# kiliant/zklaim

Measured on AMD Instinct MI355X. Metric: Groth16 proofs/sec (zklaim gadget, alt_bn128) + G1 MSM GB/s vs HBM roofline, higher is better.
Workload: dtype u32 limbs, Montgomery (254-bit Fq/Fr: 9 x 29-bit in the accumulation, reduction and NTT kernels, 8 x 32-bit elsewhere)

## Files before the change

zklaim_amd/csrc/msm.hip:

```cpp
#include "common.hpp"
#include "fq29.hip.hpp"
#include "../../include/zkg.h"
#include <algorithm>
#include <chrono>
#include <cstdio>
#include <cstdlib>
#include <cstring>
#include <mutex>

#define ZK_VGPR_CAP(n) __attribute__((amdgpu_num_vgpr((n) / 2)))
static constexpr int ACC29_VGPRS = 192;

namespace zk {

static constexpr int SCALAR_BITS = 255;
template <class F> struct RedGeom { static constexpr int LANES_LOG = sizeof(F) == sizeof(Fq) ? 7 : 6, LANES = 1 << LANES_LOG, THREADS = 4 * LANES; };
static constexpr int RED_L_LOG_TINY = 0, RED_L_LOG_SMALL = 2, RED_L_LOG_LARGE = 4;
static constexpr size_t RED_SMALL_BUCKETS = (size_t)1 << 16, RED_LARGE_BUCKETS = (size_t)1 << 18;
static constexpr int MAX_C = 16;
static constexpr uint32_t HEAVY_S = 512;
static constexpr uint32_t HEAVY_T_MAX = 1024;
static constexpr int HEAVY_PART_BLOCKS = 512, HEAVY_MERGE_BLOCKS = 128;
static constexpr int SORT_THREADS = 1024;
static constexpr int SCAN_ITEMS = 4;
// ... 253 lines not shown
    extern __shared__ uint32_t lds_u32[];
    const uint32_t s = blockIdx.x, w = blockIdx.y, t = threadIdx.x;
    const uint32_t *rel = hist + ((size_t)w * S + s) * B, *off = offsets + (size_t)w * B;
    for (uint32_t b = t; b < B; b += SORT_THREADS) lds_u32[b] = off[b] + rel[b];
    __syncthreads();
    size_t lo = (size_t)s * slice_len, hi = lo + slice_len < n ? lo + slice_len : n;
    const uint32_t *d = digits + (size_t)w * n;
    for (size_t i = lo + t; i < hi; i += SORT_THREADS) {
        uint32_t code = d[i];
        if (code) { uint32_t pos = atomicAdd(&lds_u32[(code >> 1) - 1], 1u); sorted[pos] = ((uint32_t)i << 1) | (code & 1u); }
    }
}


static constexpr uint32_t RX_MAX_CBITS = 10, RX_MAX_CB = 1u << RX_MAX_CBITS, RX_SLICE = 16384, RX_PER_THREAD = 16, RX_FINE_MAX = 8192, RX_BIN_AVG = 4096;
__global__ __launch_bounds__(1024) void k_rx_count(const uint32_t *digits, size_t n, uint32_t fbits, uint32_t cbits, uint32_t *cnt) {
    sort_wave_priority();
    __shared__ uint32_t c[RX_MAX_CB];
    const uint32_t sl = blockIdx.x, w = blockIdx.y, t = threadIdx.x, CB = 1u << cbits;
    if (t < CB) c[t] = 0;
    __syncthreads();
    size_t lo = (size_t)sl * RX_SLICE, hi = lo + RX_SLICE < n ? lo + RX_SLICE : n;
    const uint32_t *d = digits + (size_t)w * n;
    if ((n & 3) == 0) {
        for (size_t i = lo + 4 * t; i < hi; i += 4096) {
            const uint4 q = *reinterpret_cast<const uint4 *>(d + i);
            if (q.x) atomicAdd(&c[((q.x >> 1) - 1) >> fbits], 1u);
            if (q.y) atomicAdd(&c[((q.y >> 1) - 1) >> fbits], 1u);
            if (q.z) atomicAdd(&c[((q.z >> 1) - 1) >> fbits], 1u);
            if (q.w) atomicAdd(&c[((q.w >> 1) - 1) >> fbits], 1u);
        }
    } else
    for (size_t i = lo + t; i < hi; i += 1024) { uint32_t code = d[i]; if (code) atomicAdd(&c[((code >> 1) - 1) >> fbits], 1u); }
    __syncthreads();
    if (t < CB && c[t]) atomicAdd(&cnt[w * CB + t], c[t]);
}
__global__ __launch_bounds__(1024) void k_rx_scan(const uint32_t *cnt, uint32_t nbins, uint32_t *base, uint32_t *cursor, uint32_t *grand_total) {
    sort_wave_priority();
    __shared__ uint32_t part[1024];
    const uint32_t t = threadIdx.x, per = (nbins + 1023) / 1024, lo = t * per, hi = lo + per < nbins ? lo + per : nbins;
    uint32_t sum = 0;
    for (uint32_t i = lo; i < hi; ++i) sum += cnt[i];
    part[t] = sum;
    __syncthreads();
    for (uint32_t d = 1; d < 1024; d <<= 1) {
        uint32_t x = (t >= d) ? part[t - d] : 0;
        __syncthreads();
        part[t] += x;
        __syncthreads();
    }
    uint32_t run = part[t] - sum;
    for (uint32_t i = lo; i < hi; ++i) { base[i] = run; cursor[i] = 0; run += cnt[i]; }
    if (t == 1023) { base[nbins] = part[1023]; *grand_total = part[1023]; }
}
template <int T>
__global__ __launch_bounds__(T) void k_rx_scatter(const uint32_t *digits, size_t n, uint32_t fbits, uint32_t cbits, const uint32_t *base, uint32_t *cursor,
                                                   uint32_t *tmp) {
    sort_wave_priority();
    extern __shared__ uint32_t lds_u32[];
    constexpr uint32_t SLICE = RX_PER_THREAD * T;
    const uint32_t CB = 1u << cbits;
    uint32_t *stage = lds_u32, *c = lds_u32 + SLICE, *off = c + RX_MAX_CB, *gb = off + RX_MAX_CB + 1, *cur = gb + RX_MAX_CB;
    const uint32_t sl = blockIdx.x, w = blockIdx.y, t = threadIdx.x;
    for (uint32_t b = t; b < CB; b += T) c[b] = 0;
    __syncthreads();
    size_t lo = (size_t)sl * SLICE, hi = lo + SLICE < n ? lo + SLICE : n;
    const uint32_t *d = digits + (size_t)w * n;
// ... 121 lines not shown
        bufB[of[f] + atomicAdd(&cur[f], 1u)] = e & low;
    }
    __syncthreads();
    for (uint32_t p = t; p < cnt; p += T) sorted[start + p] = bufB[p];
}

ZK_D uint32_t heavy_threshold_dev(const uint32_t *offsets, size_t total_buckets, uint32_t divisor) {
    uint32_t entries = offsets[total_buckets];
    uint32_t avg6 = (uint32_t)(6 * (uint64_t)entries / total_buckets), slack = 8 + avg6 > 32 ? 32 : 8 + avg6;
    uint32_t t = (uint32_t)(4 * (uint64_t)entries / total_buckets) + slack;
    t = t > HEAVY_T_MAX ? HEAVY_T_MAX : t;
    t /= divisor;
    return t < 4 ? 4 : t;
}

__global__ __launch_bounds__(1024) void k_class_hist(const uint32_t *counts, const uint32_t *offsets, size_t total, uint32_t *class_hist) {
    sort_wave_priority();
    __shared__ uint32_t h[HEAVY_T_MAX + 2];
    const uint32_t heavy_t = heavy_threshold_dev(offsets, total, 1);
    const uint32_t t = threadIdx.x, nc = heavy_t + 2;
    for (uint32_t i = t; i < nc; i += 1024) h[i] = 0;
    __syncthreads();
    size_t gb = (size_t)blockIdx.x * 1024 + t;
    if (gb < total) { uint32_t c = counts[gb]; atomicAdd(&h[c > heavy_t ? heavy_t + 1 : c], 1u); }
    __syncthreads();
    for (uint32_t i = t; i < nc; i += 1024) if (h[i]) atomicAdd(&class_hist[i], h[i]);
}
__global__ __launch_bounds__(1024) void k_class_scan(uint32_t *class_hist, const uint32_t *offsets, size_t total) {
    sort_wave_priority();
    __shared__ uint32_t part[1024];
    const uint32_t heavy_t = heavy_threshold_dev(offsets, total, 1), nc = heavy_t + 2, t = threadIdx.x;
    uint32_t v0 = 2 * t < nc ? class_hist[nc - 1 - 2 * t] : 0, v1 = 2 * t + 1 < nc ? class_hist[nc - 2 - 2 * t] : 0;
    part[t] = v0 + v1;
    __syncthreads();
    for (uint32_t d = 1; d < 1024; d <<= 1) {
        uint32_t x = (t >= d) ? part[t - d] : 0;
        __syncthreads();
        part[t] += x;
        __syncthreads();
    }
    const uint32_t before = part[t] - v0 - v1;
    if (2 * t < nc) class_hist[nc - 1 - 2 * t] = before;
    if (2 * t + 1 < nc) class_hist[nc - 2 - 2 * t] = before + v0;
}
__global__ __launch_bounds__(1024) void k_order_place(const uint32_t *counts, const uint32_t *offsets, size_t total, uint32_t *class_cursor, uint32_t *order) {
    sort_wave_priority();
    __shared__ uint32_t h[HEAVY_T_MAX + 2];
    const uint32_t heavy_t = heavy_threshold_dev(offsets, total, 1);
    const uint32_t t = threadIdx.x, nc = heavy_t + 2;
    for (uint32_t i = t; i < nc; i += 1024) h[i] = 0;
    __syncthreads();
    size_t gb = (size_t)blockIdx.x * 1024 + t;
    uint32_t cls = 0, rank = 0;
    if (gb < total) { uint32_t c = counts[gb]; cls = c > heavy_t ? heavy_t + 1 : c; rank = atomicAdd(&h[cls], 1u); }
    __syncthreads();
    for (uint32_t i = t; i < nc; i += 1024) if (h[i]) h[i] = atomicAdd(&class_cursor[i], h[i]);
    __syncthreads();
    if (gb < total) order[h[cls] + rank] = (uint32_t)gb;
}

template <class F, bool PLAIN>
__global__ __launch_bounds__(256) void k_bucket_accum(const ViewSet<F> views, const uint32_t *sorted, const uint32_t *offsets, const uint32_t *order,
                                                       size_t lanes , XYZZ<F> *buckets, HeavyItem *items,
                                                       HeavyBucket *heavy, uint32_t *counters , SetLayout L) {
    size_t tid = (size_t)blockIdx.x * blockDim.x + threadIdx.x;
    if (tid >= lanes) return;
    const size_t total_buckets = L.buckets;
    const uint32_t set = blockIdx.y;
    const BaseView<F> bases = views.v[set];
    buckets += set * L.buckets; items += set * L.items; heavy += set * L.heavy; counters += 2 * set;
    const uint32_t heavy_t = heavy_threshold_dev(offsets, total_buckets, sizeof(F) > sizeof(Fq) ? 3 : 1);
    const uint32_t gb = order[tid];
    uint32_t k = offsets[gb], end = offsets[gb + 1];
// ... 28 lines not shown
}
ZK_D Affine29 load29(const Rec64 *bases, uint32_t e) { return load_rec64(bases + (e >> 1)); }
ZK_D Rec64 load29_raw(const Rec64 *bases, uint32_t e) { return load_rec64_raw(bases + (e >> 1)); }
template <int WAVES, bool OUT29>
__global__ __launch_bounds__(256, WAVES) ZK_VGPR_CAP(ACC29_VGPRS) void k_bucket_accum29(const Rec64 *bases, size_t level_stride, uint32_t B, const uint32_t *sorted, const uint32_t *offsets, const uint32_t *order,
                                                         size_t lanes, void *buckets_, HeavyItem *items, HeavyBucket *heavy, uint32_t *counters, SetLayout L, int flags ) {
    crit_wave_priority(flags & 2);
    const int resume = flags & 1;
    size_t tid = (size_t)blockIdx.x * blockDim.x + threadIdx.x;
    if (tid >= lanes) return;
    const uint32_t heavy_t = heavy_threshold_dev(offsets, L.buckets, 1);
    const uint32_t gb = order[tid];
    if (level_stride) bases += (size_t)(gb / B) * level_stride;
    uint32_t k = offsets[gb], end = offsets[gb + 1];
    if (end - k > heavy_t) {
        uint32_t nparts = (end - k + HEAVY_S - 1) / HEAVY_S;
        uint32_t first = atomicAdd(&counters[0], nparts);
        const bool single = nparts == 1 && !resume;
        for (uint32_t p = 0; p < nparts; ++p) { uint32_t a = k + p * HEAVY_S; items[first + p] = {a, a + HEAVY_S < end ? a + HEAVY_S : end, gb, single}; }
        if (!single) heavy[atomicAdd(&counters[1], 1u)] = {gb, first, nparts};
        return;
    }
    XYZZ29 acc; bool inf = true;
    acc.x = acc.y = acc.zz = acc.zzz = Fq29::zero();
    if constexpr (OUT29) {
        if (resume) {
            if (k >= end) return;
            const Bucket29 old = load_bucket29_raw(reinterpret_cast<const Bucket29 *>(buckets_) + gb);
            uint32_t any = 0;
#pragma unroll
// ... 542 lines not shown
};
struct MsmJob {
    hipStream_t stream = nullptr; bool own_stream = false;
    DevBuf digits, hist, counts, offsets, scan_sums, class_hist, order, sorted, rx_tmp, rx_meta;
    MsmGroup group[2];
    MsmGeom g{}; size_t n = 0;
    int window_hint = 0;
    uint32_t merge_hint = 1, merge = 1;
    hipStream_t aux = nullptr; hipEvent_t ev_fork = nullptr, ev_join = nullptr; bool converted_aside = false;
    bool one_pass_sort = false;
    bool resume = false, defer_reduce = false; bool last_out29 = false;
    hipEvent_t ev_tail = nullptr; bool tail_recorded = false;
    bool critical = false;
    MsmJob *bucket_owner = nullptr;
    hipStream_t sort_stream = nullptr; hipEvent_t ev_sorted = nullptr, ev_acc_done = nullptr;
    uint32_t w0 = 0, ws = 1;
    bool empty = false;
    uint32_t multi = 1; size_t multi_stride = 0;
    DevBuf hs_scalars; hipStream_t copy = nullptr; hipEvent_t ev_piece[8] = {nullptr};
    std::mutex mu;
};

template <class F>
static int launch_accumulate(MsmJob *job, MsmGroup &gr, const MsmBases *sets, const uint32_t *d_gather, bool time_it) {
    const MsmGeom g = job->g; const size_t n = job->n, total_buckets = (size_t)g.W * g.B; const unsigned ns = (unsigned)gr.nsets;
    const uint32_t P = job->multi, BP = g.B * P, Wp = g.W / P;
    hipStream_t s = job->stream;
    size_t n_entries_max = n * g.W;
    const size_t max_heavy = std::min(total_buckets, n_entries_max / (sizeof(F) != sizeof(Fq) ? 4 : 8)) + 1,
                 max_items = max_heavy + n_entries_max / HEAVY_S + 1;
    typedef RedGeom<F> RG;
    gr.table = sets[0].level_stride != 0;
    gr.red_windows = gr.table ? P : g.W;
    const size_t red_buckets = (size_t)gr.red_windows * g.B;
    static const char *force_l = getenv("ZKG_RED_L_LOG");
    const int red_l_log = force_l ? atoi(force_l) : red_buckets >= RED_LARGE_BUCKETS ? RED_L_LOG_LARGE : red_buckets > RED_SMALL_BUCKETS ? RED_L_LOG_SMALL : RED_L_LOG_TINY;
    gr.chunk_log = RG::LANES_LOG + red_l_log;
    gr.cpw = (g.B + (1u << gr.chunk_log) - 1) >> gr.chunk_log; gr.nred = (size_t)gr.red_windows * gr.cpw;
    DevBuf &bucket_buf = job->bucket_owner ? job->bucket_owner->group[sizeof(F) != sizeof(Fq) ? 1 : 0].buckets : gr.buckets;
    gr.red_slots = 2;
    SetLayout L; L.buckets = total_buckets; L.items = max_items; L.heavy = max_heavy; L.partials = max_items; L.folded = BP; L.red_out = gr.nred * 3;
    if (gr.heavy_items.reserve(ns * max_items * sizeof(HeavyItem)) || gr.heavy_buckets.reserve(ns * max_heavy * sizeof(HeavyBucket)) ||
        gr.heavy_counters.reserve(8 * MSM_MAX_SETS) || gr.heavy_partials.reserve(ns * max_items * sizeof(XYZZ<F>)) ||
        bucket_buf.reserve(ns * total_buckets * std::max(sizeof(XYZZ<F>), sizeof(Bucket29))) || gr.red_out.reserve(ns * L.red_out * sizeof(XYZZ<F>)) || ((gr.red_stride = L.red_out), false) ||
        (gr.table && gr.folded.reserve(ns * (size_t)BP * std::max(sizeof(XYZZ<F>), sizeof(Bucket29)))) || gr.host_reserve(ns * L.red_out * sizeof(XYZZ<F>))) return ZKG_ERROR;
// ... 19 lines not shown
                    hipLaunchKernelGGL(k_bases_to29, dim3((unsigned)((n + 255) / 256)), dim3(256), 0, s, reinterpret_cast<const Affine<Fq> *>(sets[0].p), n, gr.bases29.as<Rec64>());
                }
                rec29 = gr.bases29.as<Rec64>();
            }
        } else if (ns == 1 && !accum32 && !d_gather && sets[0].p29 && !sets[0].remap && sets[0].index_sub == 0) {
            use29 = true; rec29 = reinterpret_cast<const Rec64 *>(sets[0].p29); stride29 = sets[0].level_stride;
        }
    }
    static const bool red32_env = getenv("ZKG_REDUCE_32") != nullptr;
    static const bool fold32_env = getenv("ZKG_FOLD_32") != nullptr;
    const bool out29 = use29 && !red32_env && (stride29 == 0 ? !gr.table : (gr.table && ns == 1 && Wp <= 8 && !fold32_env));
    const int resume = job->resume ? 1 : 0;
    MsmJob *owner = job->bucket_owner ? job->bucket_owner : job;
    if (resume && !(out29 && owner->last_out29)) { set_error("msm: a piece can only continue 29-bit buckets"); return ZKG_ERROR; }
    owner->last_out29 = out29;
    if (time_it) g_dominant_timer.begin(s);
    bool done_ba = false;
    if constexpr (sizeof(F) == sizeof(Fq)) {
        const char *e_ba = getenv("ZKG_ACCUM_BA"), *e_k = getenv("ZKG_BA_K");
        const int ba_levels = e_ba ? std::max(0, std::min((int)ba::MAX_LEVELS, atoi(e_ba))) : 0;
        const int ba_k = e_k ? std::max(2, std::min(32, atoi(e_k) & ~1)) : 16;
        if (use29 && out29 && stride29 == 0 && !resume && ba_levels > 0 && n_entries_max >= 4096) {
            const int R = ba_levels, K = ba_k;
            const size_t per_wg = (size_t)ba::THREADS * K, words_start = n_entries_max / 32 + 2;
            size_t stride[ba::MAX_LEVELS + 1] = {0}, plane_words = 0, grid1 = 0;
            for (int l = 1; l <= R; ++l) {
                const size_t nodes = (n_entries_max >> l) + 1, grid = (nodes + per_wg - 1) / per_wg;
                stride[l] = grid * per_wg;
                plane_words += 18 * stride[l];
                if (l == 1) grid1 = grid;
// ... 17 lines not shown
                }
            }
            hipLaunchKernelGGL(k_bucket_accum_ba, dim3((unsigned)((lanes + 255) / 256)), dim3(256), 0, s, rec29, job->sorted.as<uint32_t>(), pl, R, job->offsets.as<uint32_t>(),
                               job->order.as<uint32_t>(), lanes, reinterpret_cast<Bucket29 *>(buckets), gr.heavy_items.as<HeavyItem>(), gr.heavy_buckets.as<HeavyBucket>(),
                               gr.heavy_counters.as<uint32_t>(), L);
            done_ba = true;
        }
    }
    if (done_ba) {}
    else if constexpr (sizeof(F) == sizeof(Fq)) {
        static const int waves_env = getenv("ZKG_ACC29_WAVES") ? atoi(getenv("ZKG_ACC29_WAVES")) : 0;
        const int waves29 = waves_env ? waves_env : (job->sort_stream || gr.table || job->bucket_owner) ? 2 : 3;
        auto launch29 = [&](auto kern) {
            hipLaunchKernelGGL(kern, dim3((unsigned)((lanes + 255) / 256)), dim3(256), 0, s, rec29, stride29, BP, job->sorted.as<uint32_t>(),
                               job->offsets.as<uint32_t>(), job->order.as<uint32_t>(), lanes, (void *)buckets, gr.heavy_items.as<HeavyItem>(),
                               gr.heavy_buckets.as<HeavyBucket>(), gr.heavy_counters.as<uint32_t>(), L, resume | (job->critical ? 2 : 0));
        };
        if (use29 && waves29 == 3) { if (out29) launch29(k_bucket_accum29<3, true>); else launch29(k_bucket_accum29<3, false>); }
        else if (use29) { if (out29) launch29(k_bucket_accum29<2, true>); else launch29(k_bucket_accum29<2, false>); }
    }
    if (use29 || done_ba) {}
    else if (plain)
        hipLaunchKernelGGL((k_bucket_accum<F, true>), dim3((unsigned)((lanes + 255) / 256), ns), dim3(256), 0, s,
                           views, job->sorted.as<uint32_t>(), job->offsets.as<uint32_t>(), job->order.as<uint32_t>(), lanes, buckets,
                           gr.heavy_items.as<HeavyItem>(), gr.heavy_buckets.as<HeavyBucket>(), gr.heavy_counters.as<uint32_t>(), L);
    else
        hipLaunchKernelGGL((k_bucket_accum<F, false>), dim3((unsigned)((lanes + 255) / 256), ns), dim3(256), 0, s,
                           views, job->sorted.as<uint32_t>(), job->offsets.as<uint32_t>(), job->order.as<uint32_t>(), lanes, buckets,
                           gr.heavy_items.as<HeavyItem>(), gr.heavy_buckets.as<HeavyBucket>(), gr.heavy_counters.as<uint32_t>(), L);
    if (time_it) g_dominant_timer.end(s);
    if (!job->defer_reduce && host_pool_prewake_enabled()) {
        if (!job->ev_tail && hipEventCreateWithFlags(&job->ev_tail, hipEventDisableTiming) != hipSuccess) job->ev_tail = nullptr;
        job->tail_recorded = job->ev_tail && hipEventRecord(job->ev_tail, s) == hipSuccess;
    }
    hipLaunchKernelGGL(k_heavy_parts<F>, dim3(HEAVY_PART_BLOCKS, ns), dim3(256), 256 * sizeof(LdsPoint<F>), s,
                       views, job->sorted.as<uint32_t>(), gr.heavy_items.as<HeavyItem>(), gr.heavy_counters.as<uint32_t>(), gr.heavy_partials.as<XYZZ<F>>(), buckets, L, (int)out29);
    hipLaunchKernelGGL(k_heavy_merge<F>, dim3(HEAVY_MERGE_BLOCKS, ns), dim3(256), 256 * sizeof(LdsPoint<F>), s,
                       gr.heavy_buckets.as<HeavyBucket>(), gr.heavy_counters.as<uint32_t>(), gr.heavy_partials.as<XYZZ<F>>(), buckets, L, (int)out29, resume);
    if (job->defer_reduce) {
        if (hipGetLastError() != hipSuccess) { set_error("msm kernel launch failed"); return ZKG_ERROR; }
        return ZKG_OK;
    }
    const XYZZ<F> *red_in = buckets; size_t in_stride = L.buckets;
    bool folded29 = false;
    if constexpr (sizeof(F) == sizeof(Fq)) {
        if (gr.table && out29) {
            hipLaunchKernelGGL(k_bucket_fold29, dim3((2 * BP + 255) / 256), dim3(256), 0, s, reinterpret_cast<const Bucket29 *>(buckets), job->counts.as<uint32_t>(), Wp, BP,
                               gr.folded.as<Bucket29>(), job->critical ? 1 : 0);
            red_in = gr.folded.as<XYZZ<F>>(); in_stride = L.folded; folded29 = true;
        }
    }
    if (gr.table && !folded29) {
        uint32_t slots = 1; while (slots < Wp && slots < 32) slots <<= 1;
// ... 106 lines not shown
    return acc;
}

static int sort_digits(MsmJob *job, const uint32_t *d_scalars, bool mont, const uint32_t *d_gather) {
    const MsmGeom g0 = job->g; const size_t n0 = job->n;
    if (job->merge > 1) { job->g.W /= job->merge; job->g.Wt = job->g.W; job->n *= job->merge; }
    if (job->multi > 1) { job->g.W *= job->multi; job->g.Wt = job->g.W; }
    const MsmGeom g = job->g; const size_t n = job->n;
    hipStream_t s = job->sort_stream ? job->sort_stream : job->stream;
    const size_t total = (size_t)g.W * g.B;
    uint32_t slice_len = (uint32_t)std::min<size_t>(65536, std::max<size_t>(4096, ((n + 15) / 16 + 1023) / 1024 * 1024));
    uint32_t S = (uint32_t)std::max<size_t>(1, (n + slice_len - 1) / slice_len);
    size_t nblk = (total + 1024 * SCAN_ITEMS - 1) / (1024 * SCAN_ITEMS);
    if (nblk > 1024) { set_error("msm: too many buckets for the block scan"); return ZKG_ERROR; }
    if (job->digits.reserve(std::max<size_t>(1, n * g.W) * 4) || job->hist.reserve((size_t)g.W * S * g.B * 4) || job->counts.reserve(total * 4) ||
        job->offsets.reserve((total + 1) * 4) || job->scan_sums.reserve(1024 * 4) || job->class_hist.reserve((HEAVY_T_MAX + 2) * 4) ||
        job->order.reserve(total * 4) || job->sorted.reserve(std::max<size_t>(1, n * g.W) * 4)) return ZKG_ERROR;
    uint32_t *digits = job->digits.as<uint32_t>(), *hist = job->hist.as<uint32_t>(), *counts = job->counts.as<uint32_t>(),
             *offsets = job->offsets.as<uint32_t>(), *sums = job->scan_sums.as<uint32_t>(), *chist = job->class_hist.as<uint32_t>();
    static const bool radix_off = getenv("ZKG_SORT_ONE_PASS") != nullptr;
    uint32_t cbits = 6;
    static const uint32_t bin_avg = getenv("ZKG_RX_AVG") ? (uint32_t)atoi(getenv("ZKG_RX_AVG")) : RX_BIN_AVG;
    while (cbits < RX_MAX_CBITS && cbits + 1 < g.c - 1 && (n >> cbits) > bin_avg) ++cbits;
    const bool two_pass = !radix_off && !job->one_pass_sort && g.c >= 12 && n >= 49152 && (n >> cbits) <= RX_FINE_MAX && n <= ((size_t)1 << (31 - (g.c - 1 - cbits)));
    {
        ZeroList zl{};
        int k = 0;
        zl.p[k] = chist; zl.words[k++] = HEAVY_T_MAX + 2;
        for (MsmGroup &gr : job->group) if (gr.nsets) {
            if (gr.heavy_counters.reserve(8 * MSM_MAX_SETS)) return ZKG_ERROR;
            zl.p[k] = gr.heavy_counters.as<uint32_t>(); zl.words[k++] = 2 * MSM_MAX_SETS;
        }
        if (two_pass) {
            const uint32_t nbins = g.W << cbits;
            if (job->rx_meta.reserve((3 * (size_t)nbins + 8) * 4)) return ZKG_ERROR;
            zl.p[k] = job->rx_meta.as<uint32_t>(); zl.words[k++] = 3 * nbins + 8;
        }
        static const bool generic_digits = getenv("ZKG_DIGITS_GENERIC") != nullptr;
        const dim3 dg((unsigned)((n0 + 255) / 256));
        const bool four = !d_gather && (n0 & 3) == 0 && g0.w0 == 0 && g0.ws == 1 && g0.W == g0.Wt;
        const dim3 dg4((unsigned)((n0 / 4 + 255) / 256));
        if (job->multi > 1) {
            const dim3 dgm(dg.x, job->multi);
            if (g0.c == 16) hipLaunchKernelGGL(k_digits_multi<16>, dgm, dim3(256), 0, s, d_scalars, job->multi_stride, n0, (int)mont, job->merge, digits, zl);
            else if (g0.c == 12) hipLaunchKernelGGL(k_digits_multi<12>, dgm, dim3(256), 0, s, d_scalars, job->multi_stride, n0, (int)mont, job->merge, digits, zl);
            else hipLaunchKernelGGL(k_digits_multi_any, dgm, dim3(256), 0, s, d_scalars, job->multi_stride, n0, (int)mont, g0, job->merge, digits, zl);
        }
        else if (!generic_digits && four && g0.c == 16) hipLaunchKernelGGL(k_digits_c4<16>, dg4, dim3(256), 0, s, d_scalars, n0, (int)mont, g0, digits, zl);
        else if (!generic_digits && four && g0.c == 12) hipLaunchKernelGGL(k_digits_c4<12>, dg4, dim3(256), 0, s, d_scalars, n0, (int)mont, g0, digits, zl);
        else if (!generic_digits && g0.c == 16) hipLaunchKernelGGL(k_digits_c<16>, dg, dim3(256), 0, s, d_scalars, d_gather, n0, (int)mont, g0, digits, zl);
        else if (!generic_digits && g0.c == 12) hipLaunchKernelGGL(k_digits_c<12>, dg, dim3(256), 0, s, d_scalars, d_gather, n0, (int)mont, g0, digits, zl);
        else hipLaunchKernelGGL(k_digits, dg, dim3(256), 0, s, d_scalars, d_gather, n0, (int)mont, g0, digits, zl);
    }
    if (two_pass) {
        const uint32_t fbits = g.c - 1 - cbits, CB = 1u << cbits, nbins = g.W * CB, S1 = (uint32_t)((n + RX_SLICE - 1) / RX_SLICE);
        if (job->rx_tmp.reserve(n * g.W * 4) || job->rx_meta.reserve((3 * (size_t)nbins + 8) * 4)) return ZKG_ERROR;
        uint32_t *cnt = job->rx_meta.as<uint32_t>(), *base = cnt + nbins, *cursor = base + nbins + 1, *tmp = job->rx_tmp.as<uint32_t>();
        hipLaunchKernelGGL(k_rx_count, dim3(S1, g.W), dim3(1024), 0, s, digits, n, fbits, cbits, cnt);
        hipLaunchKernelGGL(k_rx_scan, dim3(1), dim3(1024), 0, s, cnt, nbins, base, cursor, offsets + total);
        static const int wg_env = getenv("ZKG_SORT_WG") ? atoi(getenv("ZKG_SORT_WG")) : 0;
        const bool half = (wg_env ? wg_env == 512 : job->sort_stream != nullptr) && fbits <= 9;
        if (half) {
            const uint32_t S2 = (uint32_t)((n + 512 * RX_PER_THREAD - 1) / (512 * RX_PER_THREAD));
            hipLaunchKernelGGL(k_rx_scatter<512>, dim3(S2, g.W), dim3(512), (512 * RX_PER_THREAD + 4 * RX_MAX_CB + 8) * 4, s, digits, n, fbits, cbits, base, cursor, tmp);
            hipLaunchKernelGGL(k_rx_fine<512>, dim3(CB, g.W), dim3(512), (RX_FINE_MAX + 3 * (1u << fbits)) * 4, s, tmp, fbits, cbits, g.B, base, counts, offsets,
                               job->sorted.as<uint32_t>());
        } else {
            hipLaunchKernelGGL(k_rx_scatter<1024>, dim3(S1, g.W), dim3(1024), (RX_SLICE + 4 * RX_MAX_CB + 8) * 4, s, digits, n, fbits, cbits, base, cursor, tmp);
            hipLaunchKernelGGL(k_rx_fine<1024>, dim3(CB, g.W), dim3(1024), (RX_FINE_MAX + 3 * (1u << fbits)) * 4, s, tmp, fbits, cbits, g.B, base, counts, offsets,
                               job->sorted.as<uint32_t>());
        }
    } else {
    hipLaunchKernelGGL(k_hist, dim3(S, g.W), dim3(SORT_THREADS), g.B * 4, s, digits, n, g.B, S, slice_len, hist);
    hipLaunchKernelGGL(k_colscan, dim3((unsigned)((total + 255) / 256)), dim3(256), 0, s, hist, g.B, S, total, counts);
    hipLaunchKernelGGL(k_scan_blocks, dim3((unsigned)nblk), dim3(1024), 0, s, counts, offsets, sums, total);
    hipLaunchKernelGGL(k_scan_sums, dim3(1), dim3(1024), 0, s, sums, (uint32_t)nblk, offsets + total);
    hipLaunchKernelGGL(k_scan_apply, dim3((unsigned)nblk), dim3(1024), 0, s, offsets, sums, total);
    hipLaunchKernelGGL(k_place, dim3(S, g.W), dim3(SORT_THREADS), g.B * 4, s, digits, n, g.B, S, slice_len, hist, offsets, job->sorted.as<uint32_t>());
    }
    hipLaunchKernelGGL(k_class_hist, dim3((unsigned)((total + 1023) / 1024)), dim3(1024), 0, s, counts, offsets, total, chist);
    hipLaunchKernelGGL(k_class_scan, dim3(1), dim3(1024), 0, s, chist, offsets, total);
    hipLaunchKernelGGL(k_order_place, dim3((unsigned)((total + 1023) / 1024)), dim3(1024), 0, s, counts, offsets, total, chist, job->order.as<uint32_t>());
    if (hipGetLastError() != hipSuccess) { set_error("msm sort launch failed"); return ZKG_ERROR; }
    return ZKG_OK;
}

MsmJob *msm_job_create(hipStream_t s, bool own_stream, bool high_priority) {
    MsmJob *j = new MsmJob();
    j->stream = s;
    if (own_stream) {
        int prio_lo = 0, prio_hi = 0;
        (void)hipDeviceGetStreamPriorityRange(&prio_lo, &prio_hi);
        if (!hip_ok(hipStreamCreateWithPriority(&j->stream, hipStreamNonBlocking, high_priority ? prio_hi : prio_lo), "hipStreamCreate", __FILE__, __LINE__)) { delete j; return nullptr; }
        j->own_stream = true;
    }
    return j;
}
// ... 47 lines not shown
    {
        static const bool accum32 = getenv("ZKG_ACCUM_32") != nullptr, inline29 = getenv("ZKG_TO29_INLINE") != nullptr;
        MsmGroup &g1 = job->group[0];
        if (!accum32 && !inline29 && !any_table && !d_gather && g1.nsets == 1 && by_field[0][0].index_sub == 0 && !by_field[0][0].remap && !by_field[0][0].p29) {
            if (!job->aux && (hipStreamCreateWithFlags(&job->aux, hipStreamNonBlocking) != hipSuccess || hipEventCreateWithFlags(&job->ev_fork, hipEventDisableTiming) != hipSuccess ||
                              hipEventCreateWithFlags(&job->ev_join, hipEventDisableTiming) != hipSuccess)) { set_error("msm: side stream"); return ZKG_ERROR; }
            if (g1.bases29.reserve(n * sizeof(Rec64))) return ZKG_ERROR;
            ZK_HIP(hipEventRecord(job->ev_fork, job->stream));
            ZK_HIP(hipStreamWaitEvent(job->aux, job->ev_fork, 0));
            hipLaunchKernelGGL(k_bases_to29, dim3((unsigned)((n + 255) / 256)), dim3(256), 0, job->aux, reinterpret_cast<const Affine<Fq> *>(by_field[0][0].p), n, g1.bases29.as<Rec64>());
            ZK_HIP(hipEventRecord(job->ev_join, job->aux));
            job->converted_aside = true;
        }
    }
    auto fail = [&] { if (job->converted_aside) { (void)hipStreamSynchronize(job->aux); job->converted_aside = false; } return ZKG_ERROR; };
    if (sort_digits(job, d_scalars, scalars_mont, d_gather)) return fail();
    if (job->sort_stream && job->sort_stream != job->stream) {
        if (hipEventRecord(job->ev_sorted, job->sort_stream) != hipSuccess || hipStreamWaitEvent(job->stream, job->ev_sorted, 0) != hipSuccess) return fail();
    }
    if (job->merge > 1) {
        for (int k = 0; k < 2; ++k) for (int i = 0; i < job->group[k].nsets; ++i) by_field[k][i].level_stride *= job->merge;
    }
    lap("sort enqueued");
    const bool timed_field_g2 = job->group[0].nsets == 0;
    if (job->group[1].nsets && launch_accumulate<Fq2>(job, job->group[1], by_field[1], d_gather, job == &g_default_job && timed_field_g2)) return fail();
    if (job->group[0].nsets && launch_accumulate<Fq>(job, job->group[0], by_field[0], d_gather, job == &g_default_job || job == &g_piece_job)) return fail();
    lap("accum enqueued");
    return ZKG_OK;
}
bool msm_multi_supported(size_t n, int c, uint32_t count) {
    const MsmGeom g = pick_geom(n, c);
    return c > 0 && count >= 1 && n >= 1 && (uint64_t)n * g.W * count < ((uint64_t)1 << 31) &&
           ((uint64_t)g.W * g.B * count + 1024 * SCAN_ITEMS - 1) / (1024 * SCAN_ITEMS) <= 1024;
}
int msm_job_launch_multi(MsmJob *job, const MsmBases *sets, int nsets, const uint32_t *d_scalars, size_t n, size_t scalar_stride, uint32_t count, bool scalars_mont) {
    bool ok = job->w0 == 0 && job->ws == 1 && nsets >= 1 && nsets <= MSM_MAX_SETS && msm_multi_supported(n, job->window_hint, count);
    for (int i = 0; i < nsets && ok; ++i) ok = sets[i].level_stride != 0 && !sets[i].remap && sets[i].index_sub == 0;
    if (!ok) { set_error("msm: unsupported multi launch"); return ZKG_ERROR; }
    job->g = pick_geom(n, job->window_hint); job->n = n;
    job->empty = false; job->converted_aside = false;
    MsmBases by_field[2][MSM_MAX_SETS];
    for (MsmGroup &gr : job->group) gr.nsets = 0;
    job->group[0].g2 = false; job->group[1].g2 = true;
    for (int i = 0; i < nsets; ++i) { MsmGroup &gr = job->group[sets[i].g2 ? 1 : 0]; by_field[sets[i].g2 ? 1 : 0][gr.nsets] = sets[i]; gr.out_index[gr.nsets] = gr.nsets; ++gr.nsets; }
    job->merge = 1;
    if (job->merge_hint > 1 && job->g.W % job->merge_hint == 0) {
        bool m = true;
        for (int i = 0; i < nsets; ++i) m = m && sets[i].level_stride == n;
        if (m) job->merge = job->merge_hint;
    }
    job->multi = count; job->multi_stride = scalar_stride;
    if (sort_digits(job, d_scalars, scalars_mont, nullptr)) return ZKG_ERROR;
    for (int k = 0; k < 2; ++k) for (int i = 0; i < job->group[k].nsets; ++i) by_field[k][i].level_stride *= job->merge;
    if (job->group[1].nsets && launch_accumulate<Fq2>(job, job->group[1], by_field[1], nullptr, false)) return ZKG_ERROR;
    if (job->group[0].nsets && launch_accumulate<Fq>(job, job->group[0], by_field[0], nullptr, false)) return ZKG_ERROR;
// ... 86 lines not shown
    cut[0] = 0;
    if (const char *e = getenv("ZKG_MSM_CUTS")) {
        int k = 1; const char *q = e;
        while (*q && k < 8) { const long v = strtol(q, const_cast<char **>(&q), 10); if (v <= 0 || v >= 64) break; cut[k++] = (n * (size_t)v / 64) & ~(size_t)255; if (*q == ',') ++q; }
        if (k > 1) { P = k; cut[P] = n; for (int i = 1; i < P; ++i) if (cut[i] < cut[i - 1]) cut[i] = cut[i - 1]; }
    }
    for (int k = 0; k < P; ++k) {
        ZK_HIP(hipMemcpyAsync(d_sc + 8 * cut[k], h_scalars + 8 * cut[k], (cut[k + 1] - cut[k]) * 32, hipMemcpyHostToDevice, J.copy));
        ZK_HIP(hipEventRecord(J.ev_piece[k], J.copy));
    }
    static const bool two_jobs = getenv("ZKG_MSM_PIECES_ONE_STREAM") == nullptr;
    MsmJob &K = g_piece_job;
    if (two_jobs && !g_sort_hi) {
        int lo = 0, hi = 0; (void)hipDeviceGetStreamPriorityRange(&lo, &hi);
        bool ok = hipStreamCreateWithPriority(&g_sort_hi, hipStreamNonBlocking, hi) == hipSuccess;
        for (MsmJob *w : {&J, &K}) ok = ok && hipEventCreateWithFlags(&w->ev_sorted, hipEventDisableTiming) == hipSuccess && hipEventCreateWithFlags(&w->ev_acc_done, hipEventDisableTiming) == hipSuccess;
        if (!ok) { g_sort_hi = nullptr; set_error("msm: sort stream"); return ZKG_ERROR; }
    }
    hipStream_t s_hi = two_jobs ? g_sort_hi : nullptr;
    if (!J.aux && (hipStreamCreateWithFlags(&J.aux, hipStreamNonBlocking) != hipSuccess || hipEventCreateWithFlags(&J.ev_fork, hipEventDisableTiming) != hipSuccess ||
                   hipEventCreateWithFlags(&J.ev_join, hipEventDisableTiming) != hipSuccess)) { set_error("msm: side stream"); return ZKG_ERROR; }
    if (J.group[0].bases29.reserve(n * sizeof(Rec64))) return ZKG_ERROR;
    ZK_HIP(hipEventRecord(J.ev_fork, s));
    ZK_HIP(hipStreamWaitEvent(J.aux, J.ev_fork, 0));
    hipLaunchKernelGGL(k_bases_to29, dim3((unsigned)((n + 255) / 256)), dim3(256), 0, J.aux, reinterpret_cast<const Affine<Fq> *>(d_bases), n, J.group[0].bases29.as<Rec64>());
    ZK_HIP(hipEventRecord(J.ev_join, J.aux));
    ZK_HIP(hipStreamWaitEvent(s, J.ev_join, 0));
    if (s_hi) ZK_HIP(hipStreamWaitEvent(s_hi, J.ev_fork, 0));
    const int c = (int)pick_geom(n, J.window_hint).c;
    const int saved_hint = J.window_hint, saved_hint_k = K.window_hint;
    J.window_hint = c; K.window_hint = c; K.bucket_owner = &J; K.w0 = 0; K.ws = 1; K.one_pass_sort = false; K.stream = s;
    int rc = ZKG_OK; bool started = false; bool used[2] = {false, false};
    for (int k = 0; k < P && rc == ZKG_OK; ++k) {
        if (cut[k + 1] == cut[k] && k + 1 < P) continue;
        const int which = (two_jobs && ((P - 1 - k) & 1)) ? 1 : 0;
        MsmJob &W = which ? K : J;
        MsmBases piece = set; piece.p = reinterpret_cast<const char *>(d_bases) + cut[k] * sizeof(G1Affine);
        piece.p29 = J.group[0].bases29.as<Rec64>() + cut[k];
        W.resume = started; W.defer_reduce = k + 1 < P; started = true;
        W.sort_stream = s_hi;
        hipStream_t ss = s_hi ? s_hi : s;
        if (hipStreamWaitEvent(ss, J.ev_piece[k], 0) != hipSuccess) { rc = ZKG_ERROR; break; }
        if (s_hi && used[which] && hipStreamWaitEvent(s_hi, W.ev_acc_done, 0) != hipSuccess) { rc = ZKG_ERROR; break; }
        rc = msm_job_launch(&W, &piece, 1, d_sc + 8 * cut[k], cut[k + 1] - cut[k], mont, nullptr);
        if (rc == ZKG_OK && s_hi && hipEventRecord(W.ev_acc_done, s) != hipSuccess) rc = ZKG_ERROR;
        used[which] = true;
    }
    J.resume = false; J.defer_reduce = false; J.window_hint = saved_hint; J.sort_stream = nullptr;
    K.resume = false; K.defer_reduce = false; K.window_hint = saved_hint_k; K.bucket_owner = nullptr; K.sort_stream = nullptr; K.stream = nullptr;
    if (rc != ZKG_OK) { (void)hipStreamSynchronize(J.copy); if (s_hi) (void)hipStreamSynchronize(s_hi); (void)hipStreamSynchronize(s); return ZKG_ERROR; }
    return msm_job_finish(&J, out, nullptr);
}

int msm_g1(const G1Affine *d_bases, const uint32_t *d_scalars, size_t n, bool mont, G1 *out, hipStream_t s, bool mostly_bits) {
    return msm_shared(&d_bases, 1, nullptr, d_scalars, n, mont, out, nullptr, s, 0, 1, mostly_bits);
}
int msm_g2(const G2Affine *d_bases, const uint32_t *d_scalars, size_t n, bool mont, G2 *out, hipStream_t s, bool mostly_bits) {
    return msm_shared(nullptr, 0, d_bases, d_scalars, n, mont, nullptr, out, s, 0, 1, mostly_bits);
}

template <class F>
// ... 190 lines not shown
    for (auto &gr : j.group) gr.release();
    if (j.aux) { (void)hipStreamSynchronize(j.aux); (void)hipStreamDestroy(j.aux); j.aux = nullptr; }
    j.hs_scalars.release();
    {
        MsmJob &k = g_piece_job;
        if (g_sort_hi) { (void)hipStreamSynchronize(g_sort_hi); (void)hipStreamDestroy(g_sort_hi); g_sort_hi = nullptr; }
        for (DevBuf *b : {&k.digits, &k.hist, &k.counts, &k.offsets, &k.scan_sums, &k.class_hist, &k.order, &k.sorted, &k.rx_tmp, &k.rx_meta}) b->release();
        for (auto &gr : k.group) gr.release();
        if (k.aux) { (void)hipStreamSynchronize(k.aux); (void)hipStreamDestroy(k.aux); k.aux = nullptr; }
        if (k.ev_fork) { (void)hipEventDestroy(k.ev_fork); k.ev_fork = nullptr; }
        if (k.ev_tail) { (void)hipEventDestroy(k.ev_tail); k.ev_tail = nullptr; k.tail_recorded = false; }
        if (k.ev_join) { (void)hipEventDestroy(k.ev_join); k.ev_join = nullptr; }
        for (MsmJob *w : {&j, &k}) {
            if (w->ev_sorted) { (void)hipEventDestroy(w->ev_sorted); w->ev_sorted = nullptr; }
            if (w->ev_acc_done) { (void)hipEventDestroy(w->ev_acc_done); w->ev_acc_done = nullptr; }
        }
        k.stream = nullptr;
    }
    if (j.copy) { (void)hipStreamSynchronize(j.copy); (void)hipStreamDestroy(j.copy); j.copy = nullptr; }
    for (auto &e : j.ev_piece) if (e) { (void)hipEventDestroy(e); e = nullptr; }
    if (j.ev_fork) { (void)hipEventDestroy(j.ev_fork); j.ev_fork = nullptr; }
    if (j.ev_tail) { (void)hipEventDestroy(j.ev_tail); j.ev_tail = nullptr; j.tail_recorded = false; }
    if (j.ev_join) { (void)hipEventDestroy(j.ev_join); j.ev_join = nullptr; }
}

}
```

Baseline: 56.92.

## Fuse sort scans into last-workgroup tails and run heavy buckets on sort stream

Folds the single-block scan kernels (rx_scan, class_scan) into the tail of the preceding histogram kernels using an atomic ticket, so the last workgroup does the scan. This removes two kernel launches and their dependencies. k_order_place now also builds the heavy-bucket item lists during the sort. For piecewise G1 MSMs with a separate high-priority sort stream, the heavy-bucket parts and merge kernels run on the sort stream concurrently with the light-bucket accumulation, and the accumulation skips heavy buckets. The cost is extra events and cross-stream ordering, which risks races on the shared bucket buffers.

After: 55.92. 1.8% lower.

```diff
diff --git a/zklaim_amd/csrc/msm.hip b/zklaim_amd/csrc/msm.hip
--- a/zklaim_amd/csrc/msm.hip
+++ b/zklaim_amd/csrc/msm.hip
@@ -291,9 +291,18 @@
 
 
 static constexpr uint32_t RX_MAX_CBITS = 10, RX_MAX_CB = 1u << RX_MAX_CBITS, RX_SLICE = 16384, RX_PER_THREAD = 16, RX_FINE_MAX = 8192, RX_BIN_AVG = 4096;
-__global__ __launch_bounds__(1024) void k_rx_count(const uint32_t *digits, size_t n, uint32_t fbits, uint32_t cbits, uint32_t *cnt) {
+ZK_D uint32_t ld_agent(const uint32_t *p) { return __hip_atomic_load(p, __ATOMIC_RELAXED, __HIP_MEMORY_SCOPE_AGENT); }
+ZK_D bool last_workgroup(uint32_t *ticket, uint32_t *verdict ) {
+    __syncthreads();
+    if (threadIdx.x == 0) *verdict = __hip_atomic_fetch_add(ticket, 1u, __ATOMIC_ACQ_REL, __HIP_MEMORY_SCOPE_AGENT) == gridDim.x * gridDim.y - 1;
+    __syncthreads();
+    return *verdict != 0;
+}
+__global__ __launch_bounds__(1024) void k_rx_count(const uint32_t *digits, size_t n, uint32_t fbits, uint32_t cbits, uint32_t *cnt, uint32_t nbins, uint32_t *base,
+                                                    uint32_t *cursor, uint32_t *grand_total, uint32_t *ticket) {
     sort_wave_priority();
     __shared__ uint32_t c[RX_MAX_CB];
+    __shared__ uint32_t last;
     const uint32_t sl = blockIdx.x, w = blockIdx.y, t = threadIdx.x, CB = 1u << cbits;
     if (t < CB) c[t] = 0;
     __syncthreads();
@@ -311,13 +320,11 @@
     for (size_t i = lo + t; i < hi; i += 1024) { uint32_t code = d[i]; if (code) atomicAdd(&c[((code >> 1) - 1) >> fbits], 1u); }
     __syncthreads();
     if (t < CB && c[t]) atomicAdd(&cnt[w * CB + t], c[t]);
-}
-__global__ __launch_bounds__(1024) void k_rx_scan(const uint32_t *cnt, uint32_t nbins, uint32_t *base, uint32_t *cursor, uint32_t *grand_total) {
-    sort_wave_priority();
-    __shared__ uint32_t part[1024];
-    const uint32_t t = threadIdx.x, per = (nbins + 1023) / 1024, lo = t * per, hi = lo + per < nbins ? lo + per : nbins;
+    if (!last_workgroup(ticket, &last)) return;
+    uint32_t *part = c;
+    const uint32_t per = (nbins + 1023) / 1024, blo = t * per, bhi = blo + per < nbins ? blo + per : nbins;
     uint32_t sum = 0;
-    for (uint32_t i = lo; i < hi; ++i) sum += cnt[i];
+    for (uint32_t i = blo; i < bhi; ++i) sum += ld_agent(cnt + i);
     part[t] = sum;
     __syncthreads();
     for (uint32_t d = 1; d < 1024; d <<= 1) {
@@ -327,7 +334,7 @@
         __syncthreads();
     }
     uint32_t run = part[t] - sum;
-    for (uint32_t i = lo; i < hi; ++i) { base[i] = run; cursor[i] = 0; run += cnt[i]; }
+    for (uint32_t i = blo; i < bhi; ++i) { base[i] = run; cursor[i] = 0; run += ld_agent(cnt + i); }
     if (t == 1023) { base[nbins] = part[1023]; *grand_total = part[1023]; }
 }
 template <int T>
@@ -479,7 +486,36 @@
     return t < 4 ? 4 : t;
 }
 
+static constexpr uint32_t CLASS_TICKET = HEAVY_T_MAX + 2, CLASS_WORDS = HEAVY_T_MAX + 3;
 __global__ __launch_bounds__(1024) void k_class_hist(const uint32_t *counts, const uint32_t *offsets, size_t total, uint32_t *class_hist) {
+    sort_wave_priority();
+    __shared__ uint32_t h[HEAVY_T_MAX + 2];
+    __shared__ uint32_t last;
+    const uint32_t heavy_t = heavy_threshold_dev(offsets, total, 1);
+    const uint32_t t = threadIdx.x, nc = heavy_t + 2;
+    for (uint32_t i = t; i < nc; i += 1024) h[i] = 0;
+    __syncthreads();
+    size_t gb = (size_t)blockIdx.x * 1024 + t;
+    if (gb < total) { uint32_t c = counts[gb]; atomicAdd(&h[c > heavy_t ? heavy_t + 1 : c], 1u); }
+    __syncthreads();
+    for (uint32_t i = t; i < nc; i += 1024) if (h[i]) atomicAdd(&class_hist[i], h[i]);
+    if (!last_workgroup(class_hist + CLASS_TICKET, &last)) return;
+    uint32_t *part = h;
+    uint32_t v0 = 2 * t < nc ? ld_agent(class_hist + (nc - 1 - 2 * t)) : 0, v1 = 2 * t + 1 < nc ? ld_agent(class_hist + (nc - 2 - 2 * t)) : 0;
+    part[t] = v0 + v1;
+    __syncthreads();
+    for (uint32_t d = 1; d < 1024; d <<= 1) {
+        uint32_t x = (t >= d) ? part[t - d] : 0;
+        __syncthreads();
+        part[t] += x;
+        __syncthreads();
+    }
+    const uint32_t before = part[t] - v0 - v1;
+    if (2 * t < nc) class_hist[nc - 1 - 2 * t] = before;
+    if (2 * t + 1 < nc) class_hist[nc - 2 - 2 * t] = before + v0;
+}
+__global__ __launch_bounds__(1024) void k_order_place(const uint32_t *counts, const uint32_t *offsets, size_t total, uint32_t *class_cursor, uint32_t *order,
+                                                       HeavyItem *items, HeavyBucket *heavy, uint32_t *counters, int resume) {
     sort_wave_priority();
     __shared__ uint32_t h[HEAVY_T_MAX + 2];
     const uint32_t heavy_t = heavy_threshold_dev(offsets, total, 1);
@@ -487,41 +523,19 @@
     for (uint32_t i = t; i < nc; i += 1024) h[i] = 0;
     __syncthreads();
     size_t gb = (size_t)blockIdx.x * 1024 + t;
-    if (gb < total) { uint32_t c = counts[gb]; atomicAdd(&h[c > heavy_t ? heavy_t + 1 : c], 1u); }
-    __syncthreads();
-    for (uint32_t i = t; i < nc; i += 1024) if (h[i]) atomicAdd(&class_hist[i], h[i]);
-}
-__global__ __launch_bounds__(1024) void k_class_scan(uint32_t *class_hist, const uint32_t *offsets, size_t total) {
-    sort_wave_priority();
-    __shared__ uint32_t part[1024];
-    const uint32_t heavy_t = heavy_threshold_dev(offsets, total, 1), nc = heavy_t + 2, t = threadIdx.x;
-    uint32_t v0 = 2 * t < nc ? class_hist[nc - 1 - 2 * t] : 0, v1 = 2 * t + 1 < nc ? class_hist[nc - 2 - 2 * t] : 0;
-    part[t] = v0 + v1;
-    __syncthreads();
-    for (uint32_t d = 1; d < 1024; d <<= 1) {
-        uint32_t x = (t >= d) ? part[t - d] : 0;
-        __syncthreads();
-        part[t] += x;
-        __syncthreads();
-    }
-    const uint32_t before = part[t] - v0 - v1;
-    if (2 * t < nc) class_hist[nc - 1 - 2 * t] = before;
-    if (2 * t + 1 < nc) class_hist[nc - 2 - 2 * t] = before + v0;
-}
-__global__ __launch_bounds__(1024) void k_order_place(const uint32_t *counts, const uint32_t *offsets, size_t total, uint32_t *class_cursor, uint32_t *order) {
-    sort_wave_priority();
-    __shared__ uint32_t h[HEAVY_T_MAX + 2];
-    const uint32_t heavy_t = heavy_threshold_dev(offsets, total, 1);
-    const uint32_t t = threadIdx.x, nc = heavy_t + 2;
-    for (uint32_t i = t; i < nc; i += 1024) h[i] = 0;
-    __syncthreads();
-    size_t gb = (size_t)blockIdx.x * 1024 + t;
     uint32_t cls = 0, rank = 0;
     if (gb < total) { uint32_t c = counts[gb]; cls = c > heavy_t ? heavy_t + 1 : c; rank = atomicAdd(&h[cls], 1u); }
     __syncthreads();
     for (uint32_t i = t; i < nc; i += 1024) if (h[i]) h[i] = atomicAdd(&class_cursor[i], h[i]);
     __syncthreads();
     if (gb < total) order[h[cls] + rank] = (uint32_t)gb;
+    if (items && gb < total && cls == heavy_t + 1) {
+        const uint32_t k = offsets[gb], end = offsets[gb + 1], nparts = (end - k + HEAVY_S - 1) / HEAVY_S;
+        const uint32_t first = atomicAdd(&counters[0], nparts);
+        const bool single = nparts == 1 && !resume;
+        for (uint32_t p = 0; p < nparts; ++p) { uint32_t a = k + p * HEAVY_S; items[first + p] = {a, a + HEAVY_S < end ? a + HEAVY_S : end, (uint32_t)gb, single}; }
+        if (!single) heavy[atomicAdd(&counters[1], 1u)] = {(uint32_t)gb, first, nparts};
+    }
 }
 
 template <class F, bool PLAIN>
@@ -580,6 +594,7 @@
     if (level_stride) bases += (size_t)(gb / B) * level_stride;
     uint32_t k = offsets[gb], end = offsets[gb + 1];
     if (end - k > heavy_t) {
+        if (flags & 4) return;
         uint32_t nparts = (end - k + HEAVY_S - 1) / HEAVY_S;
         uint32_t first = atomicAdd(&counters[0], nparts);
         const bool single = nparts == 1 && !resume;
@@ -1152,6 +1167,7 @@
     bool critical = false;
     MsmJob *bucket_owner = nullptr;
     hipStream_t sort_stream = nullptr; hipEvent_t ev_sorted = nullptr, ev_acc_done = nullptr;
+    bool heavy_aside = false; hipEvent_t ev_prev_acc = nullptr, ev_heavy_done = nullptr; const void *heavy_items_at_sort = nullptr;
     uint32_t w0 = 0, ws = 1;
     bool empty = false;
     uint32_t multi = 1; size_t multi_stride = 0;
@@ -1159,14 +1175,19 @@
     std::mutex mu;
 };
 
+template <class F> static void heavy_capacity(size_t total_buckets, size_t n_entries_max, size_t *max_heavy, size_t *max_items) {
+    *max_heavy = std::min(total_buckets, n_entries_max / (sizeof(F) != sizeof(Fq) ? 4 : 8)) + 1;
+    *max_items = *max_heavy + n_entries_max / HEAVY_S + 1;
+}
+
 template <class F>
 static int launch_accumulate(MsmJob *job, MsmGroup &gr, const MsmBases *sets, const uint32_t *d_gather, bool time_it) {
     const MsmGeom g = job->g; const size_t n = job->n, total_buckets = (size_t)g.W * g.B; const unsigned ns = (unsigned)gr.nsets;
     const uint32_t P = job->multi, BP = g.B * P, Wp = g.W / P;
     hipStream_t s = job->stream;
     size_t n_entries_max = n * g.W;
-    const size_t max_heavy = std::min(total_buckets, n_entries_max / (sizeof(F) != sizeof(Fq) ? 4 : 8)) + 1,
-                 max_items = max_heavy + n_entries_max / HEAVY_S + 1;
+    size_t max_heavy, max_items;
+    heavy_capacity<F>(total_buckets, n_entries_max, &max_heavy, &max_items);
     typedef RedGeom<F> RG;
     gr.table = sets[0].level_stride != 0;
     gr.red_windows = gr.table ? P : g.W;
@@ -1216,6 +1237,20 @@
     MsmJob *owner = job->bucket_owner ? job->bucket_owner : job;
     if (resume && !(out29 && owner->last_out29)) { set_error("msm: a piece can only continue 29-bit buckets"); return ZKG_ERROR; }
     owner->last_out29 = out29;
+    const bool aside = job->heavy_aside;
+    if (aside) {
+        if (!(use29 && out29 && ns == 1 && job->ev_sorted)) { set_error("msm: heavy buckets beside the accumulation need a plain 29-bit G1 piece"); return ZKG_ERROR; }
+        hipStream_t sh = job->sort_stream;
+        if (gr.heavy_items.p != job->heavy_items_at_sort) { set_error("msm: heavy lists moved after the sort"); return ZKG_ERROR; }
+        hipLaunchKernelGGL(k_heavy_parts<F>, dim3(HEAVY_PART_BLOCKS, ns), dim3(256), 256 * sizeof(LdsPoint<F>), sh,
+                           views, job->sorted.as<uint32_t>(), gr.heavy_items.as<HeavyItem>(), gr.heavy_counters.as<uint32_t>(), gr.heavy_partials.as<XYZZ<F>>(), buckets, L, (int)out29);
+        ZK_HIP(hipEventRecord(job->ev_sorted, sh));
+        ZK_HIP(hipStreamWaitEvent(s, job->ev_sorted, 0));
+        if (job->ev_prev_acc) ZK_HIP(hipStreamWaitEvent(sh, job->ev_prev_acc, 0));
+        hipLaunchKernelGGL(k_heavy_merge<F>, dim3(HEAVY_MERGE_BLOCKS, ns), dim3(256), 256 * sizeof(LdsPoint<F>), sh,
+                           gr.heavy_buckets.as<HeavyBucket>(), gr.heavy_counters.as<uint32_t>(), gr.heavy_partials.as<XYZZ<F>>(), buckets, L, (int)out29, resume);
+        if (!job->defer_reduce) ZK_HIP(hipEventRecord(job->ev_heavy_done, sh));
+    }
     if (time_it) g_dominant_timer.begin(s);
     bool done_ba = false;
     if constexpr (sizeof(F) == sizeof(Fq)) {
@@ -1263,7 +1298,7 @@
         auto launch29 = [&](auto kern) {
             hipLaunchKernelGGL(kern, dim3((unsigned)((lanes + 255) / 256)), dim3(256), 0, s, rec29, stride29, BP, job->sorted.as<uint32_t>(),
                                job->offsets.as<uint32_t>(), job->order.as<uint32_t>(), lanes, (void *)buckets, gr.heavy_items.as<HeavyItem>(),
-                               gr.heavy_buckets.as<HeavyBucket>(), gr.heavy_counters.as<uint32_t>(), L, resume | (job->critical ? 2 : 0));
+                               gr.heavy_buckets.as<HeavyBucket>(), gr.heavy_counters.as<uint32_t>(), L, resume | (job->critical ? 2 : 0) | (aside ? 4 : 0));
         };
         if (use29 && waves29 == 3) { if (out29) launch29(k_bucket_accum29<3, true>); else launch29(k_bucket_accum29<3, false>); }
         else if (use29) { if (out29) launch29(k_bucket_accum29<2, true>); else launch29(k_bucket_accum29<2, false>); }
@@ -1282,10 +1317,13 @@
         if (!job->ev_tail && hipEventCreateWithFlags(&job->ev_tail, hipEventDisableTiming) != hipSuccess) job->ev_tail = nullptr;
         job->tail_recorded = job->ev_tail && hipEventRecord(job->ev_tail, s) == hipSuccess;
     }
+    if (aside) { if (!job->defer_reduce) ZK_HIP(hipStreamWaitEvent(s, job->ev_heavy_done, 0)); }
+    else {
     hipLaunchKernelGGL(k_heavy_parts<F>, dim3(HEAVY_PART_BLOCKS, ns), dim3(256), 256 * sizeof(LdsPoint<F>), s,
                        views, job->sorted.as<uint32_t>(), gr.heavy_items.as<HeavyItem>(), gr.heavy_counters.as<uint32_t>(), gr.heavy_partials.as<XYZZ<F>>(), buckets, L, (int)out29);
     hipLaunchKernelGGL(k_heavy_merge<F>, dim3(HEAVY_MERGE_BLOCKS, ns), dim3(256), 256 * sizeof(LdsPoint<F>), s,
                        gr.heavy_buckets.as<HeavyBucket>(), gr.heavy_counters.as<uint32_t>(), gr.heavy_partials.as<XYZZ<F>>(), buckets, L, (int)out29, resume);
+    }
     if (job->defer_reduce) {
         if (hipGetLastError() != hipSuccess) { set_error("msm kernel launch failed"); return ZKG_ERROR; }
         return ZKG_OK;
@@ -1422,7 +1460,7 @@
     size_t nblk = (total + 1024 * SCAN_ITEMS - 1) / (1024 * SCAN_ITEMS);
     if (nblk > 1024) { set_error("msm: too many buckets for the block scan"); return ZKG_ERROR; }
     if (job->digits.reserve(std::max<size_t>(1, n * g.W) * 4) || job->hist.reserve((size_t)g.W * S * g.B * 4) || job->counts.reserve(total * 4) ||
-        job->offsets.reserve((total + 1) * 4) || job->scan_sums.reserve(1024 * 4) || job->class_hist.reserve((HEAVY_T_MAX + 2) * 4) ||
+        job->offsets.reserve((total + 1) * 4) || job->scan_sums.reserve(1024 * 4) || job->class_hist.reserve(CLASS_WORDS * 4) ||
         job->order.reserve(total * 4) || job->sorted.reserve(std::max<size_t>(1, n * g.W) * 4)) return ZKG_ERROR;
     uint32_t *digits = job->digits.as<uint32_t>(), *hist = job->hist.as<uint32_t>(), *counts = job->counts.as<uint32_t>(),
              *offsets = job->offsets.as<uint32_t>(), *sums = job->scan_sums.as<uint32_t>(), *chist = job->class_hist.as<uint32_t>();
@@ -1434,7 +1472,7 @@
     {
         ZeroList zl{};
         int k = 0;
-        zl.p[k] = chist; zl.words[k++] = HEAVY_T_MAX + 2;
+        zl.p[k] = chist; zl.words[k++] = CLASS_WORDS;
         for (MsmGroup &gr : job->group) if (gr.nsets) {
             if (gr.heavy_counters.reserve(8 * MSM_MAX_SETS)) return ZKG_ERROR;
             zl.p[k] = gr.heavy_counters.as<uint32_t>(); zl.words[k++] = 2 * MSM_MAX_SETS;
@@ -1464,8 +1502,7 @@
         const uint32_t fbits = g.c - 1 - cbits, CB = 1u << cbits, nbins = g.W * CB, S1 = (uint32_t)((n + RX_SLICE - 1) / RX_SLICE);
         if (job->rx_tmp.reserve(n * g.W * 4) || job->rx_meta.reserve((3 * (size_t)nbins + 8) * 4)) return ZKG_ERROR;
         uint32_t *cnt = job->rx_meta.as<uint32_t>(), *base = cnt + nbins, *cursor = base + nbins + 1, *tmp = job->rx_tmp.as<uint32_t>();
-        hipLaunchKernelGGL(k_rx_count, dim3(S1, g.W), dim3(1024), 0, s, digits, n, fbits, cbits, cnt);
-        hipLaunchKernelGGL(k_rx_scan, dim3(1), dim3(1024), 0, s, cnt, nbins, base, cursor, offsets + total);
+        hipLaunchKernelGGL(k_rx_count, dim3(S1, g.W), dim3(1024), 0, s, digits, n, fbits, cbits, cnt, nbins, base, cursor, offsets + total, cnt + 3 * nbins + 4);
         static const int wg_env = getenv("ZKG_SORT_WG") ? atoi(getenv("ZKG_SORT_WG")) : 0;
         const bool half = (wg_env ? wg_env == 512 : job->sort_stream != nullptr) && fbits <= 9;
         if (half) {
@@ -1487,8 +1524,11 @@
     hipLaunchKernelGGL(k_place, dim3(S, g.W), dim3(SORT_THREADS), g.B * 4, s, digits, n, g.B, S, slice_len, hist, offsets, job->sorted.as<uint32_t>());
     }
     hipLaunchKernelGGL(k_class_hist, dim3((unsigned)((total + 1023) / 1024)), dim3(1024), 0, s, counts, offsets, total, chist);
-    hipLaunchKernelGGL(k_class_scan, dim3(1), dim3(1024), 0, s, chist, offsets, total);
-    hipLaunchKernelGGL(k_order_place, dim3((unsigned)((total + 1023) / 1024)), dim3(1024), 0, s, counts, offsets, total, chist, job->order.as<uint32_t>());
+    {
+        MsmGroup &g1 = job->group[0];
+        hipLaunchKernelGGL(k_order_place, dim3((unsigned)((total + 1023) / 1024)), dim3(1024), 0, s, counts, offsets, total, chist, job->order.as<uint32_t>(),
+                           job->heavy_aside ? g1.heavy_items.as<HeavyItem>() : nullptr, g1.heavy_buckets.as<HeavyBucket>(), g1.heavy_counters.as<uint32_t>(), job->resume ? 1 : 0);
+    }
     if (hipGetLastError() != hipSuccess) { set_error("msm sort launch failed"); return ZKG_ERROR; }
     return ZKG_OK;
 }
@@ -1566,8 +1606,17 @@
         }
     }
     auto fail = [&] { if (job->converted_aside) { (void)hipStreamSynchronize(job->aux); job->converted_aside = false; } return ZKG_ERROR; };
+    job->heavy_aside = false;
+    if (job->sort_stream && job->sort_stream != job->stream && job->ev_heavy_done && !any_table && !d_gather && job->group[1].nsets == 0 && job->group[0].nsets == 1 &&
+        by_field[0][0].p29 && !(getenv("ZKG_ACCUM_BA") && atoi(getenv("ZKG_ACCUM_BA")) > 0)) {
+        MsmGroup &g1 = job->group[0];
+        size_t max_heavy, max_items;
+        heavy_capacity<Fq>((size_t)job->g.W * job->g.B, n * job->g.W, &max_heavy, &max_items);
+        if (g1.heavy_items.reserve(max_items * sizeof(HeavyItem)) || g1.heavy_buckets.reserve(max_heavy * sizeof(HeavyBucket))) return fail();
+        job->heavy_aside = true; job->heavy_items_at_sort = g1.heavy_items.p;
+    }
     if (sort_digits(job, d_scalars, scalars_mont, d_gather)) return fail();
-    if (job->sort_stream && job->sort_stream != job->stream) {
+    if (job->sort_stream && job->sort_stream != job->stream && !job->heavy_aside) {
         if (hipEventRecord(job->ev_sorted, job->sort_stream) != hipSuccess || hipStreamWaitEvent(job->stream, job->ev_sorted, 0) != hipSuccess) return fail();
     }
     if (job->merge > 1) {
@@ -1590,7 +1639,7 @@
     for (int i = 0; i < nsets && ok; ++i) ok = sets[i].level_stride != 0 && !sets[i].remap && sets[i].index_sub == 0;
     if (!ok) { set_error("msm: unsupported multi launch"); return ZKG_ERROR; }
     job->g = pick_geom(n, job->window_hint); job->n = n;
-    job->empty = false; job->converted_aside = false;
+    job->empty = false; job->converted_aside = false; job->heavy_aside = false;
     MsmBases by_field[2][MSM_MAX_SETS];
     for (MsmGroup &gr : job->group) gr.nsets = 0;
     job->group[0].g2 = false; job->group[1].g2 = true;
@@ -1707,7 +1756,8 @@
     if (two_jobs && !g_sort_hi) {
         int lo = 0, hi = 0; (void)hipDeviceGetStreamPriorityRange(&lo, &hi);
         bool ok = hipStreamCreateWithPriority(&g_sort_hi, hipStreamNonBlocking, hi) == hipSuccess;
-        for (MsmJob *w : {&J, &K}) ok = ok && hipEventCreateWithFlags(&w->ev_sorted, hipEventDisableTiming) == hipSuccess && hipEventCreateWithFlags(&w->ev_acc_done, hipEventDisableTiming) == hipSuccess;
+        for (MsmJob *w : {&J, &K}) ok = ok && hipEventCreateWithFlags(&w->ev_sorted, hipEventDisableTiming) == hipSuccess && hipEventCreateWithFlags(&w->ev_acc_done, hipEventDisableTiming) == hipSuccess &&
+                                        hipEventCreateWithFlags(&w->ev_heavy_done, hipEventDisableTiming) == hipSuccess;
         if (!ok) { g_sort_hi = nullptr; set_error("msm: sort stream"); return ZKG_ERROR; }
     }
     hipStream_t s_hi = two_jobs ? g_sort_hi : nullptr;
@@ -1723,7 +1773,7 @@
     const int c = (int)pick_geom(n, J.window_hint).c;
     const int saved_hint = J.window_hint, saved_hint_k = K.window_hint;
     J.window_hint = c; K.window_hint = c; K.bucket_owner = &J; K.w0 = 0; K.ws = 1; K.one_pass_sort = false; K.stream = s;
-    int rc = ZKG_OK; bool started = false; bool used[2] = {false, false};
+    int rc = ZKG_OK; bool started = false; bool used[2] = {false, false}; MsmJob *prev = nullptr;
     for (int k = 0; k < P && rc == ZKG_OK; ++k) {
         if (cut[k + 1] == cut[k] && k + 1 < P) continue;
         const int which = (two_jobs && ((P - 1 - k) & 1)) ? 1 : 0;
@@ -1732,12 +1782,13 @@
         piece.p29 = J.group[0].bases29.as<Rec64>() + cut[k];
         W.resume = started; W.defer_reduce = k + 1 < P; started = true;
         W.sort_stream = s_hi;
+        W.ev_prev_acc = (s_hi && prev) ? prev->ev_acc_done : nullptr;
         hipStream_t ss = s_hi ? s_hi : s;
         if (hipStreamWaitEvent(ss, J.ev_piece[k], 0) != hipSuccess) { rc = ZKG_ERROR; break; }
         if (s_hi && used[which] && hipStreamWaitEvent(s_hi, W.ev_acc_done, 0) != hipSuccess) { rc = ZKG_ERROR; break; }
         rc = msm_job_launch(&W, &piece, 1, d_sc + 8 * cut[k], cut[k + 1] - cut[k], mont, nullptr);
         if (rc == ZKG_OK && s_hi && hipEventRecord(W.ev_acc_done, s) != hipSuccess) rc = ZKG_ERROR;
-        used[which] = true;
+        used[which] = true; prev = &W;
     }
     J.resume = false; J.defer_reduce = false; J.window_hint = saved_hint; J.sort_stream = nullptr;
     K.resume = false; K.defer_reduce = false; K.window_hint = saved_hint_k; K.bucket_owner = nullptr; K.sort_stream = nullptr; K.stream = nullptr;
@@ -1958,6 +2009,7 @@
         for (MsmJob *w : {&j, &k}) {
             if (w->ev_sorted) { (void)hipEventDestroy(w->ev_sorted); w->ev_sorted = nullptr; }
             if (w->ev_acc_done) { (void)hipEventDestroy(w->ev_acc_done); w->ev_acc_done = nullptr; }
+            if (w->ev_heavy_done) { (void)hipEventDestroy(w->ev_heavy_done); w->ev_heavy_done = nullptr; }
         }
         k.stream = nullptr;
     }
```
